# BornToDeath/h264-h265-to-jpeg

Hardware: AMD Instinct MI355X
Metric: 1080p H.265 I-frames/sec → JPEG at 1/2/4/8 MI355X; achieved HBM GB/s vs peak (higher is better)
Workload: dtype u8

## Files before the change

### h264-h265-to-jpeg_amd/csrc/host/bitstream.cpp

```cpp
#include "bitstream.h"

namespace h2j {

void split_annexb(const uint8_t* d, size_t n, std::vector<Nal>& out) {
    out.clear();
    size_t i = 0;
    long start = -1;
    while (i + 2 < n) {
        if (d[i + 2] > 1) {
            i += 3;
            continue;
        }
        if (d[i] == 0 && d[i + 1] == 0 && d[i + 2] == 1) {
            if (start >= 0) {
                size_t e = i;
                while (e > static_cast<size_t>(start) && d[e - 1] == 0) e--;
                out.push_back(Nal{d + start, e - start});
            }
            i += 3;
            start = static_cast<long>(i);
            continue;
        }
        i++;
    }
    if (start >= 0 && static_cast<size_t>(start) < n) {
        size_t e = n;
        while (e > static_cast<size_t>(start) && d[e - 1] == 0) e--;
        out.push_back(Nal{d + start, e - start});
    }
}

size_t unescape_rbsp(const uint8_t* src, size_t n, uint8_t* dst) {
    size_t o = 0;
    int zeros = 0;
    for (size_t i = 0; i < n; i++) {
        uint8_t b = src[i];
        if (zeros >= 2 && b == 3) {
            zeros = 0;
            continue;
        }
        dst[o++] = b;
        zeros = (b == 0) ? zeros + 1 : 0;
    }
    return o;
}

bool BitReader::more_rbsp_data() const {
    long last = static_cast<long>(n_) - 1;
    while (last >= 0 && p_[last] == 0) last--;
    if (last < 0) return false;
    int tz = 0;
    while (!((p_[last] >> tz) & 1)) tz++;
    size_t stop = static_cast<size_t>(last) * 8 + (7 - tz);
    return pos_ < stop;
}

int detect_codec(const uint8_t* d, size_t n) {
    std::vector<Nal> nals;
    split_annexb(d, n < (1u << 16) ? n : (1u << 16), nals);
    int hv = 0, hs = 0, hp = 0, as = 0, ap = 0;
    for (const Nal& nal : nals) {
        if (nal.n < 2) continue;
        uint8_t h0 = nal.p[0], h1 = nal.p[1];
        if (h0 & 0x80) continue;
        int t = (h0 >> 1) & 63, layer = ((h0 & 1) << 5) | (h1 >> 3), tid = h1 & 7;
        if (layer == 0 && tid >= 1) {
            if (t == 32) hv++;
            if (t == 33) hs++;
            if (t == 34) hp++;
        }
        int t4 = h0 & 31;
        if (t4 == 7) as++;
        if (t4 == 8) ap++;
    }
    if (hv && hs && hp) return 265;
    if (as && ap) return 264;
    return 0;
}

int sei_display_orientation(const uint8_t* rbsp, size_t n, bool hevc, int cur) {
    static const uint8_t kCode[2][2][4] = {{{0, 8, 3, 6}, {4, 7, 2, 5}}, {{2, 5, 4, 7}, {3, 6, 0, 8}}};
    (void)hevc;
    size_t pos = 0;
    while (n - pos >= 2) {
        uint32_t type = 0, size = 0;
        while (pos < n && rbsp[pos] == 0xFF && type < (1u << 20)) { type += 255; pos++; }
        if (pos >= n) break;
        type += rbsp[pos++];
        while (pos < n && rbsp[pos] == 0xFF && size < (1u << 20)) { size += 255; pos++; }
        if (pos >= n) {
            if (type == 47) cur = 0;
            break;
        }
        size += rbsp[pos++];
        if (size > n - pos) {
// ... 41 lines not shown
```

### h264-h265-to-jpeg_amd/csrc/host/cabac.h

```cpp
#pragma once
#include <cstdint>

namespace h2j {

#ifdef H2J_CABAC_COUNT
extern thread_local unsigned long long g_bins_ctx, g_bins_byp;
#define H2J_COUNT(v, n) (v += (n))
struct ResidualStats {
    unsigned long long tbs, sb_visited, csbf_bins, sb_coded, sig_bins, sig0_bins, gt1_bins, gt2_bins, last_bins,
        coefs, sb_by_coefs[5] , rem_coefs, rem_sbs, sign_batch_sbs, sign_single_sbs;
    unsigned long long one_coef, one_coef_esc, one_coef_esc_price, one_coef_tskip, one_coef_bypass, one_coef_esc_tskip,
        one_coef_esc_bypass, dc_last_sb, dc_only_tb, sign_pair;
};
extern thread_local ResidualStats g_rstat;
#define H2J_STAT(f, n) (g_rstat.f += (n))
#else
#define H2J_COUNT(v, n) ((void)0)
#define H2J_STAT(f, n) ((void)0)
#endif

#pragma GCC visibility push(hidden)
extern const uint8_t kCabacLps[64][4];
extern const uint8_t kCabacTransLps[64];
extern const uint8_t kCabacRenorm[32];
extern const uint16_t kCabacNextMps[128];
extern const uint16_t kCabacNextLps[128];
extern const uint8_t kCabacLpsByState[128][8];
typedef uint64_t CabacState;
extern const uint64_t kCabacWord[128];

extern const uint64_t kCabacNextMpsW[128];
extern const uint64_t kCabacNextLpsW[128];
#pragma GCC visibility pop


inline uint8_t cabac_init_state(int m, int n, int qp) {
    if (qp < 0) qp = 0;
    if (qp > 51) qp = 51;
    int pre = ((m * qp) >> 4) + n;
    if (pre < 1) pre = 1;
    if (pre > 126) pre = 126;
    int mps = pre <= 63 ? 0 : 1;
    int st = mps ? pre - 64 : 63 - pre;
    return static_cast<uint8_t>((st << 1) | mps);
}
inline CabacState cabac_init_word(int m, int n, int qp) { return kCabacWord[cabac_init_state(m, n, qp)]; }

template <bool kInlineRefill>
class CabacT {
public:
    void init(const uint8_t* p, const uint8_t* end) {
        cur_ = p;
        end_ = end;
        range_ = 510;
        value_ = 0;
        for (int i = 0; i < 4; i++) value_ = (value_ << 8) | (cur_ < end_ ? *cur_++ : 0u);
        bits_ = 32 - 9;
    }
    __attribute__((always_inline)) inline int decision(CabacState& ctx) {
        H2J_COUNT(g_bins_ctx, 1);
        const uint64_t w = ctx;
        const unsigned st = static_cast<unsigned>(w >> 32);
        const uint32_t lps = static_cast<uint32_t>(w >> ((range_ >> 3) & 24)) & 0xffu;
        const uint32_t rmps = range_ - lps;
        const uint64_t scaled = static_cast<uint64_t>(rmps) << bits_;
        const uint32_t msh = (rmps >> 8) ^ 1u;
        uint32_t r = rmps << msh, sh = msh;
        const uint32_t lsh = static_cast<uint32_t>(__builtin_clz(lps)) - 23u;
        const uint32_t lr = lps << lsh;
        uint64_t nx = kCabacNextMpsW[st];
        const uint64_t nl = kCabacNextLpsW[st];
        uint64_t v = value_;
        const uint64_t vl = value_ - scaled;
        uint32_t is_lps = 0;
#if defined(__x86_64__)
        __asm__("cmpq %[sc], %[v]\n\t"
                "cmovaeq %[vl], %[v]\n\t"
                "cmovael %[lr], %[r]\n\t"
                "cmovael %[ls], %[sh]\n\t"
                "cmovaeq %[nl], %[nx]\n\t"
                "setae %b[il]"
                : [v] "+r"(v), [r] "+r"(r), [sh] "+r"(sh), [nx] "+r"(nx), [il] "+q"(is_lps)
                : [sc] "r"(scaled), [vl] "r"(vl), [lr] "r"(lr), [ls] "r"(lsh), [nl] "r"(nl)
                : "cc");
#else
        is_lps = v >= scaled ? 1u : 0u;
        v = is_lps ? vl : v;
        r = is_lps ? lr : r;
        sh = is_lps ? lsh : sh;
        nx = is_lps ? nl : nx;
#endif
        value_ = v;
        range_ = r;
        bits_ -= static_cast<int>(sh);
        ctx = nx;
        if (bits_ < 0) refill();
        return static_cast<int>((st & 1) ^ is_lps);
    }
    __attribute__((always_inline)) int bypass_b() {
        H2J_COUNT(g_bins_byp, 1);
        if (--bits_ < 0) refill();
        const uint64_t scaled = static_cast<uint64_t>(range_) << bits_;
        const bool one = value_ >= scaled;
        value_ -= one ? scaled : 0;
        return one;
    }
    __attribute__((always_inline)) uint32_t bypass_batch_b(int k) {
        H2J_COUNT(g_bins_byp, k);
        if (bits_ < k) refill();
        const int sh = bits_ - k;
        const uint64_t v = value_ >> sh;
        const uint32_t q = static_cast<uint32_t>(v / range_);
        value_ -= (static_cast<uint64_t>(q) * range_) << sh;
        bits_ = sh;
        return q;
    }
    __attribute__((always_inline)) uint32_t bypass_peek_b(int k) {
        if (bits_ < k) refill();
        return static_cast<uint32_t>((value_ >> (bits_ - k)) / range_);
    }
    __attribute__((always_inline)) void bypass_skip_b(int n, uint32_t top) {
        H2J_COUNT(g_bins_byp, n);
        const int sh = bits_ - n;
        value_ -= (static_cast<uint64_t>(top) * range_) << sh;
        bits_ = sh;
    }
    __attribute__((always_inline)) uint32_t bypass_bits_b(int n) {
        if (n <= 2) {
            uint32_t v = 0;
            for (int i = 0; i < n; i++) v = (v << 1) | static_cast<uint32_t>(bypass());
            return v;
        }
        if (n <= 24) return bypass_batch(n);
        const uint32_t hi = bypass_batch(n - 16);
        return (hi << 16) | bypass_batch(16);
    }
    __attribute__((always_inline)) int terminate_b() {
        range_ -= 2;
        const uint64_t scaled = static_cast<uint64_t>(range_) << bits_;
        if (value_ >= scaled) return 1;
        if (range_ < 256) {
            range_ <<= 1;
            if (--bits_ < 0) refill();
        }
        return 0;
    }
    __attribute__((always_inline)) int bypass() { return kInlineRefill ? bypass_b() : bypass_o(); }
    int bypass_o() { return bypass_b(); }
    __attribute__((always_inline)) uint32_t bypass_batch(int k) { return kInlineRefill ? bypass_batch_b(k) : bypass_batch_o(k); }
    uint32_t bypass_batch_o(int k) { return bypass_batch_b(k); }
    __attribute__((always_inline)) uint32_t bypass_peek(int k) { return kInlineRefill ? bypass_peek_b(k) : bypass_peek_o(k); }
    uint32_t bypass_peek_o(int k) { return bypass_peek_b(k); }
    __attribute__((always_inline)) void bypass_skip(int n, uint32_t top) { kInlineRefill ? bypass_skip_b(n, top) : bypass_skip_o(n, top); }
    void bypass_skip_o(int n, uint32_t top) { bypass_skip_b(n, top); }
    __attribute__((always_inline)) uint32_t bypass_bits(int n) { return kInlineRefill ? bypass_bits_b(n) : bypass_bits_o(n); }
    uint32_t bypass_bits_o(int n) { return bypass_bits_b(n); }
    __attribute__((always_inline)) int terminate() { return kInlineRefill ? terminate_b() : terminate_o(); }
    int terminate_o() { return terminate_b(); }
    const uint8_t* aligned_pos() const { return cur_ - (bits_ >> 3); }

private:
    __attribute__((always_inline)) void refill() {
        if (kInlineRefill) refill_word();
        else refill_o();
    }
    void refill_o() {
        uint32_t w;
        if (end_ - cur_ >= 4) {
            w = (static_cast<uint32_t>(cur_[0]) << 24) | (static_cast<uint32_t>(cur_[1]) << 16) |
                (static_cast<uint32_t>(cur_[2]) << 8) | cur_[3];
            cur_ += 4;
        } else {
            w = 0;
            for (int i = 0; i < 4; i++) w = (w << 8) | (cur_ < end_ ? *cur_++ : 0u);
        }
        value_ = (value_ << 32) | w;
        bits_ += 32;
    }
    __attribute__((always_inline)) void refill_word() {
        uint32_t w;
        if (__builtin_expect(end_ - cur_ >= 4, 1)) {
            w = (static_cast<uint32_t>(cur_[0]) << 24) | (static_cast<uint32_t>(cur_[1]) << 16) |
                (static_cast<uint32_t>(cur_[2]) << 8) | cur_[3];
            cur_ += 4;
        } else {
            w = tail_word(cur_, end_);
            cur_ = end_ > cur_ ? end_ : cur_;
        }
        value_ = (value_ << 32) | w;
        bits_ += 32;
    }
    __attribute__((noinline)) static uint32_t tail_word(const uint8_t* cur, const uint8_t* end) {
        uint32_t w = 0;
        for (int i = 0; i < 4; i++) w = (w << 8) | (cur < end ? *cur++ : 0u);
        return w;
    }
    const uint8_t* cur_ = nullptr;
    const uint8_t* end_ = nullptr;
    uint64_t value_ = 0;
    uint32_t range_ = 510;
    int bits_ = 0;
};
typedef CabacT<true> Cabac;
typedef CabacT<false> CabacOutlineRefill;

}
```

### h264-h265-to-jpeg_amd/csrc/host/hevc_parser.cpp

```cpp
#include <algorithm>
#include <array>
#include <atomic>
#include <cstdlib>
#include <cstring>
#include <memory>
#include <thread>
#include <vector>

#include "bitstream.h"
#include "cabac.h"
#include "job.h"

namespace h2j {
namespace {

enum {
    C_SAO_MERGE = 0, C_SAO_TYPE = 1, C_SPLIT_CU = 2, C_TQ_BYPASS = 5, C_PART_MODE = 6,
    C_PREV_INTRA = 7, C_CHROMA_MODE = 8, C_SPLIT_TF = 9, C_CBF_LUMA = 12, C_CBF_CHROMA = 14,
    C_TSKIP = 18, C_LAST_X = 20, C_LAST_Y = 38, C_CSBF = 56, C_SIG = 60, C_GT1 = 104,
    C_GT2 = 128, C_QP_DELTA = 134, C_CQO_FLAG = 136, C_CQO_IDX = 137, NUM_CTX = 138
};

const uint8_t kInitI[NUM_CTX] = {
    153, 200, 139, 141, 157, 154, 184, 184, 63, 153, 138, 138, 111, 141, 94, 138, 182, 154,
// ... 974 lines not shown
}

const uint8_t kSigTs[2][16] = {{C_SIG + 42, C_SIG + 42, C_SIG + 42, C_SIG + 42, C_SIG + 42, C_SIG + 42, C_SIG + 42, C_SIG + 42,
                                C_SIG + 42, C_SIG + 42, C_SIG + 42, C_SIG + 42, C_SIG + 42, C_SIG + 42, C_SIG + 42, C_SIG + 42},
                               {C_SIG + 43, C_SIG + 43, C_SIG + 43, C_SIG + 43, C_SIG + 43, C_SIG + 43, C_SIG + 43, C_SIG + 43,
                                C_SIG + 43, C_SIG + 43, C_SIG + 43, C_SIG + 43, C_SIG + 43, C_SIG + 43, C_SIG + 43, C_SIG + 43}};

__attribute__((always_inline)) inline int read_remaining(Cabac& cc, int rice) {
    constexpr int kPeek = 20;
    const uint32_t q = cc.bypass_peek(kPeek);
    const uint32_t inv = ~q << (32 - kPeek);
    int prefix = inv ? __builtin_clz(inv) : kPeek;
    if (prefix < kPeek) {
        const int slen = prefix < 3 ? rice : prefix - 3 + rice, total = prefix + 1 + slen;
        if (total <= kPeek) {
            const uint32_t top = q >> (kPeek - total);
            cc.bypass_skip(total, top);
            const int suf = static_cast<int>(top & ((1u << slen) - 1u));
            return prefix < 3 ? (prefix << rice) + suf : (((1 << (prefix - 3)) + 2) << rice) + suf;
        }
    }
    prefix = 0;
    while (prefix < 32 && cc.bypass()) prefix++;
    if (prefix < 3) return (prefix << rice) + static_cast<int>(cc.bypass_bits(rice));
    const int pm3 = prefix - 3;
    if (pm3 + rice > 30) return -1;
    return (((1 << pm3) + 2) << rice) + static_cast<int>(cc.bypass_bits(pm3 + rice));
}

__attribute__((noinline)) int HevcParser::remaining_level(int rice) { return read_remaining(cc_, rice); }

template <bool RExt>
void HevcParser::residual(int log2n, int c, int pred_mode, h2j_tu& tu) {
    Cabac cc = cc_;
    CabacState* const ctx = ctx_;
    const int n = 1 << log2n;
    if (p_->transform_skip && !cu_bypass_ && log2n <= (RExt ? p_->log2_max_ts : 2) && cc.decision(ctx[C_TSKIP + (c ? 1 : 0)]))
        tu.flags |= H2J_TU_TSKIP;
    const bool tsb = (tu.flags & H2J_TU_TSKIP) != 0 || cu_bypass_;
    const bool ts_ctx = RExt && s_->ts_context && tsb;
    const bool no_sdh = RExt && s_->implicit_rdpcm && (tu.flags & H2J_TU_TSKIP) && (pred_mode == 10 || pred_mode == 26);
    const bool price = RExt && s_->persistent_rice;
    int* const stat = &stat_[2 * (c == 0 ? 1 : 0) + (tsb ? 1 : 0)];
    int off, shift;
    if (c == 0) {
        off = 3 * (log2n - 2) + ((log2n - 1) >> 2);
        shift = (log2n + 1) >> 2;
    } else {
        off = 15;
        shift = log2n - 2;
    }
    const int maxp = (log2n << 1) - 1;
    H2J_STAT(tbs, 1);
    auto last_prefix = [&](CabacState* lc) __attribute__((always_inline)) {
        int k = 0, pk = 0;
        CabacState pw = lc[0];
        while (k < maxp) {
            const int ci = k >> shift;
            const CabacState lw = lc[ci];
            lc[pk] = pw;
            CabacState w = ci == pk ? pw : lw;
            H2J_STAT(last_bins, 1);
            const int b = cc.decision(w);
            pw = w;
            pk = ci;
            if (!b) break;
            k++;
        }
        lc[pk] = pw;
        return k;
    };
    int lx = last_prefix(ctx + C_LAST_X + off);
    int ly = last_prefix(ctx + C_LAST_Y + off);
    if (lx > 3) {
        int nb = (lx >> 1) - 1;
        lx = (1 << nb) * (2 + (lx & 1)) + static_cast<int>(cc.bypass_bits(nb));
    }
    if (ly > 3) {
        int nb = (ly >> 1) - 1;
        ly = (1 << nb) * (2 + (ly & 1)) + static_cast<int>(cc.bypass_bits(nb));
    }
    int scanIdx = 0;
    if (log2n == 2 || (log2n == 3 && c == 0)) {
        if (pred_mode >= 6 && pred_mode <= 14) scanIdx = 2;
        else if (pred_mode >= 22 && pred_mode <= 30) scanIdx = 1;
    }
    if (scanIdx == 2) std::swap(lx, ly);
    if (lx >= n || ly >= n) { err_ = -20; cc_ = cc; return; }
    const uint8_t(*sc)[64][2] = scanIdx == 0 ? g_scan_diag : (scanIdx == 1 ? g_scan_hor : g_scan_ver);
    const int lsb = log2n - 2;
    const int lastSub = g_scan_inv[scanIdx][lsb][((ly >> 2) << lsb) + (lx >> 2)];
    const int lastPos = g_scan_inv[scanIdx][2][((ly & 3) << 2) + (lx & 3)];
    uint64_t csbm = 0;
    H2J_STAT(dc_only_tb, (lx | ly) == 0);
    int greater1_ctx = 1;
    const bool sdh = p_->sign_hiding != 0;
    uint32_t out[32 * 32];
    int nout = 0;
    const uint16_t* const posTab = g_scan_off[scanIdx][lsb];
    const uint8_t(*const sigtab)[2][16] = g_sigctx[c ? 1 : 0][lsb][scanIdx];
    CabacState* const gt1ctx = ctx + C_GT1 + (c ? 16 : 0);
    for (int i = lastSub; i >= 0; i--) {
        const int xs = sc[lsb][i][0], ys = sc[lsb][i][1];
        H2J_STAT(sb_visited, 1);
        bool infer_dc = false;
        const int sp = ys * 8 + xs;
        const unsigned csr = static_cast<unsigned>(((csbm >> 1) & 0x7f7f7f7f7f7f7f7full) >> sp) & 1u;
        const unsigned csb = static_cast<unsigned>((csbm >> 8) >> sp) & 1u;
        unsigned coded = 1;
        if (i < lastSub && i > 0) {
            H2J_STAT(csbf_bins, 1);
            coded = static_cast<unsigned>(cc.decision(ctx[C_CSBF + (csr | csb) + (c ? 2 : 0)]));
            infer_dc = true;
        }
        csbm |= static_cast<uint64_t>(coded) << sp;
        const int prevCsbf = static_cast<int>(csr | (csb << 1));
        unsigned sigmask = 0;
        int nstart = 15;
        if (i == lastSub) {
            nstart = lastPos - 1;
            sigmask = 1u << lastPos;
            H2J_STAT(dc_last_sb, lastPos == 0);
        }
        if (coded && nstart >= 0) {
            const uint8_t* sig = ts_ctx ? kSigTs[c ? 1 : 0] : sigtab[prevCsbf][(xs | ys) ? 1 : 0];
            unsigned got = 0;
            if (nstart > 0) {
                H2J_STAT(sig_bins, nstart);
                int pidx = sig[nstart];
                CabacState pw = ctx[pidx];
                got = static_cast<unsigned>(cc.decision(pw)) << nstart;
                for (int nn = nstart - 1; nn > 0; nn--) {
                    const int idx = sig[nn];
                    const CabacState lw = ctx[idx];
                    ctx[pidx] = pw;
                    CabacState w = idx == pidx ? pw : lw;
                    got |= static_cast<unsigned>(cc.decision(w)) << nn;
                    pw = w;
                    pidx = idx;
                }
                ctx[pidx] = pw;
            }
            sigmask |= got;
            if (infer_dc && got == 0) {
                sigmask |= 1u;
            } else {
                H2J_STAT(sig0_bins, 1);
                if (cc.decision(ctx[sig[0]])) sigmask |= 1u;
            }
        }
        if (!sigmask) continue;
        H2J_STAT(sb_coded, 1);
        int ctxSet = (i == 0 || c > 0) ? 0 : 2;
        if (greater1_ctx == 0) ctxSet++;
        const int sb_off = ((ys << 2) << log2n) + (xs << 2);
#ifdef H2J_CABAC_COUNT
        {
            const int nc = __builtin_popcount(sigmask);
            H2J_STAT(coefs, nc);
            H2J_STAT(sb_by_coefs[nc == 1 ? 0 : nc == 2 ? 1 : nc == 3 ? 2 : nc < 8 ? 3 : 4], 1);
            H2J_STAT(gt1_bins, nc < 8 ? nc : 8);
        }
#endif
        if ((sigmask & (sigmask - 1)) == 0) {
            H2J_STAT(one_coef, 1);
            H2J_STAT(sign_single_sbs, 1);
            H2J_STAT(one_coef_tskip, (tu.flags & H2J_TU_TSKIP) != 0);
            H2J_STAT(one_coef_bypass, cu_bypass_ != 0);
            const int g1 = cc.decision(gt1ctx[ctxSet * 4 + 1]);
            greater1_ctx = g1 ^ 1;
            int lvl = 1 + g1, g2 = 0;
            if (g1) {
                H2J_STAT(gt2_bins, 1);
                g2 = cc.decision(ctx[C_GT2 + ctxSet + (c ? 4 : 0)]);
                lvl += g2;
            }
            const int neg = cc.bypass();
            if (g2) {
                H2J_STAT(one_coef_esc, 1);
                H2J_STAT(one_coef_esc_price, price);
                H2J_STAT(one_coef_esc_tskip, (tu.flags & H2J_TU_TSKIP) != 0);
                H2J_STAT(one_coef_esc_bypass, cu_bypass_ != 0);
                H2J_STAT(rem_coefs, 1);
                H2J_STAT(rem_sbs, 1);
                cc_ = cc;
                const int rem = remaining_level(price ? *stat / 4 : 0);
                cc = cc_;
                if (rem < 0) { err_ = -21; return; }
                lvl += rem;
                if (price) {
                    const int ri = *stat / 4;
                    if (rem >= (3 << ri)) ++*stat;
                    else if (2 * rem < (1 << ri) && *stat > 0) --*stat;
                }
            }
            int v = neg ? -lvl : lvl;
            if (v > 32767) v = 32767;
            if (v < -32768) v = -32768;
            out[nout++] = (static_cast<uint32_t>(sb_off + posTab[__builtin_ctz(sigmask)]) << 16) | static_cast<uint16_t>(v);
            continue;
        }
        greater1_ctx = 1;
        unsigned g1mask = 0;
        int numG1 = 0, lastG1 = -1;
        unsigned m_uncoded = 0;
        const int lastSig = 31 - __builtin_clz(sigmask), firstSig = __builtin_ctz(sigmask);
        CabacState* const g1c = gt1ctx + ctxSet * 4;
        {
            CabacState w0 = g1c[0], w1 = g1c[1], w2 = g1c[2], w3 = g1c[3];
            unsigned seen = 0, m = sigmask;
            auto bin = [&](CabacState& slot) __attribute__((always_inline)) {
                const int nn = 31 - __builtin_clz(m);
                m &= ~(1u << nn);
                CabacState w = seen ? w0 : slot;
                const unsigned d = static_cast<unsigned>(cc.decision(w));
                if (seen) w0 = w;
                else slot = w;
                seen |= d;
                g1mask |= d << nn;
                numG1++;
            };
            if (m) bin(w1);
            if (m) bin(w2);
            while (m && numG1 < 8) bin(w3);
            g1c[0] = w0;
            g1c[1] = w1;
            g1c[2] = w2;
            g1c[3] = w3;
            m_uncoded = m;
            greater1_ctx = seen ? 0 : 1;
        }
        if (g1mask) lastG1 = 31 - __builtin_clz(g1mask);
        const bool hidden = !cu_bypass_ && !no_sdh && (lastSig - firstSig > 3);
        int g2 = 0;
        if (lastG1 != -1) {
            H2J_STAT(gt2_bins, 1);
            g2 = cc.decision(ctx[C_GT2 + ctxSet + (c ? 4 : 0)]);
        }
        const unsigned signed_mask = (sdh && hidden) ? (sigmask & ~(1u << firstSig)) : sigmask;
        const int ns = __builtin_popcount(signed_mask);
        H2J_STAT(sign_batch_sbs, ns > 1);
        H2J_STAT(sign_single_sbs, ns <= 1);
        H2J_STAT(sign_pair, ns == 2);
        const uint32_t q = ns > 2 ? cc.bypass_batch(ns) : cc.bypass_bits(ns);
        uint32_t qs = ns ? q << (32 - ns) : 0u;
        unsigned esc = g1mask | m_uncoded;
        if (lastG1 >= 0 && !g2) esc &= ~(1u << lastG1);
        H2J_STAT(rem_coefs, __builtin_popcount(esc));
        H2J_STAT(rem_sbs, esc != 0);
        int remv[16] = {};
        int rice = price ? *stat / 4 : 0;
        bool stat_done = false;
        for (unsigned e = esc; e;) {
            const int nn = 31 - __builtin_clz(e);
            e &= ~(1u << nn);
            const int baseL = 1 + ((g1mask >> nn) & 1) + (nn == lastG1 ? g2 : 0);
            const int rem = read_remaining(cc, rice);
            if (rem < 0) { err_ = -21; cc_ = cc; return; }
            remv[nn] = rem;
            if (baseL + rem > 3 * (1 << rice)) rice = price ? rice + 1 : (rice < 4 ? rice + 1 : 4);
            if (price && !stat_done) {
                const int ri = *stat / 4;
                if (rem >= (3 << ri)) ++*stat;
                else if (2 * rem < (1 << ri) && *stat > 0) --*stat;
                stat_done = true;
            }
        }
        const int flip_last = (sdh && hidden) ? 1 : 0;
        int sumAbs = 0;
        for (unsigned mm = sigmask; mm;) {
            const int nn = 31 - __builtin_clz(mm);
            mm &= ~(1u << nn);
            const int lvl = 1 + ((g1mask >> nn) & 1) + (nn == lastG1 ? g2 : 0) + remv[nn];
            sumAbs += lvl;
            const int neg = static_cast<int>(qs >> 31) ^ (mm == 0 ? (flip_last & sumAbs) : 0);
            qs <<= 1;
            int v = neg ? -lvl : lvl;
            if (v > 32767) v = 32767;
            if (v < -32768) v = -32768;
            out[nout++] = (static_cast<uint32_t>(sb_off + posTab[nn]) << 16) | static_cast<uint16_t>(v);
        }
    }
    cc_ = cc;
    const uint32_t base = static_cast<uint32_t>(job_->coefs.size());
    job_->coefs.insert(job_->coefs.end(), out, out + nout);
    tu.coef = base - job_->hdr.coef;
    tu.ncoef = static_cast<uint16_t>(nout);
    tu.flags |= H2J_TU_CBF;
}

void HevcParser::split_ctb_records(size_t first) {
    std::vector<h2j_tu>& v = job_->tus;
    chroma_tmp_.clear();
    size_t w = first;
    for (size_t i = first; i < v.size(); i++) {
        if (v[i].c == 0) v[w++] = v[i];
        else chroma_tmp_.push_back(v[i]);
    }
    std::copy(chroma_tmp_.begin(), chroma_tmp_.end(), v.begin() + static_cast<long>(w));
}

void HevcParser::emit_tu(int x, int y, int log2n, int c, int mode, uint8_t flags, bool cbf, int) {
    job_->tus.emplace_back();
    h2j_tu& tu = job_->tus.back();
    tu.x = static_cast<uint16_t>(x);
    tu.y = static_cast<uint16_t>(y);
    tu.log2n = static_cast<uint8_t>(log2n);
    tu.c = static_cast<uint8_t>(c);
    tu.mode = static_cast<uint8_t>(mode);
    tu.flags = flags;
    tu.qp = 0;
    tu.qpy = 0;
    tu.ncoef = 0;
    tu.coef = 0;
    if (cbf) {
        if (rext_) residual<true>(log2n, c, mode, tu);
        else residual<false>(log2n, c, mode, tu);
    }
}

void HevcParser::transform_unit(int x0, int y0, int xb, int yb, int log2n, int blk, int cbf_l, int cbf_cb,
                                int cbf_cr, int cm, int cux, int cuy, int log2cb) {
    if ((cbf_l || cbf_cb || cbf_cr) && p_->cu_qp_delta && !is_qpd_coded_) {
        int v = 0;
        if (dec(C_QP_DELTA)) {
            v = 1;
            while (v < 5 && dec(C_QP_DELTA + 1)) v++;
            if (v == 5) {
                int k = 0;
                while (k < 32 && cc_.bypass()) k++;
                if (k > 30) { err_ = -22; return; }
                v += ((1 << k) - 1) + static_cast<int>(cc_.bypass_bits(k));
            }
        }
        if (v && cc_.bypass()) v = -v;
        is_qpd_coded_ = true;
        qpd_val_ = v;
        qp_y_ = qp_wrap(qg_pred_ + v + 52 + 2 * qpbd) - qpbd;
        set_qp(cux, cuy, 1 << log2cb, qp_y_);
    }
    if ((cbf_cb || cbf_cr) && cur_->cu_chroma_qp_offset_enabled && !cu_bypass_ && !cqo_coded_) {
        int idx = -1;
        if (dec(C_CQO_FLAG)) {
            idx = 0;
            if (p_->cqo_len_minus1 > 0)
                while (idx < 5 && dec(C_CQO_IDX)) idx++;
        }
        cu_qo_cb_ = idx < 0 ? 0 : p_->cb_qo[idx];
        cu_qo_cr_ = idx < 0 ? 0 : p_->cr_qo[idx];
        cqo_coded_ = true;
    }
    const int lmode = ipm_[(y0 >> 2) * mw + (x0 >> 2)];
    uint8_t fl = edge_flags(x0, y0);
    if (cu_bypass_) fl |= H2J_TU_BYPASS | H2J_TU_NOFILT;
    uint8_t lfl = fl;
    if (log2n == 2) lfl |= H2J_TU_DST;
    emit_tu(x0, y0, log2n, 0, lmode, lfl, cbf_l != 0, lmode);
    if ((job_->tus.back().flags & (H2J_TU_TSKIP | H2J_TU_BYPASS)) != 0) job_->tus.back().flags &= ~H2J_TU_DST;
    if (err_) return;
    uint8_t cfl = cu_bypass_ ? (H2J_TU_BYPASS | H2J_TU_NOFILT) : 0;
    if (log2n > 2) {
        emit_tu(x0 >> 1, y0 >> 1, log2n - 1, 1, cm, cfl, cbf_cb != 0, cm);
        if (err_) return;
        emit_tu(x0 >> 1, y0 >> 1, log2n - 1, 2, cm, cfl, cbf_cr != 0, cm);
    } else if (blk == 3) {
        emit_tu(xb >> 1, yb >> 1, 2, 1, cm, cfl, cbf_cb != 0, cm);
        if (err_) return;
        emit_tu(xb >> 1, yb >> 1, 2, 2, cm, cfl, cbf_cr != 0, cm);
    }
}

void HevcParser::transform_tree(int x0, int y0, int xb, int yb, int log2n, int depth, int blk, int max_depth,
                                int intra_split, int pcb, int pcr, int cm, int cux, int cuy, int log2cb) {
    if (err_) return;
    int split;
    if (log2n <= s_->log2_max_tb && log2n > s_->log2_min_tb && depth < max_depth && !(intra_split && depth == 0))
        split = dec(C_SPLIT_TF + 5 - log2n);
    else
        split = log2n > s_->log2_max_tb || (intra_split && depth == 0);
    int cbf_cb = 0, cbf_cr = 0;
    if (log2n > 2) {
        if (depth == 0 || pcb) cbf_cb = dec(C_CBF_CHROMA + depth);
        if (depth == 0 || pcr) cbf_cr = dec(C_CBF_CHROMA + depth);
    } else {
        cbf_cb = pcb;
        cbf_cr = pcr;
    }
    if (split) {
        if (log2n <= 2) { err_ = -23; return; }
        int h = 1 << (log2n - 1);
        transform_tree(x0, y0, x0, y0, log2n - 1, depth + 1, 0, max_depth, intra_split, cbf_cb, cbf_cr, cm, cux, cuy, log2cb);
        transform_tree(x0 + h, y0, x0, y0, log2n - 1, depth + 1, 1, max_depth, intra_split, cbf_cb, cbf_cr, cm, cux, cuy, log2cb);
        transform_tree(x0, y0 + h, x0, y0, log2n - 1, depth + 1, 2, max_depth, intra_split, cbf_cb, cbf_cr, cm, cux, cuy, log2cb);
        transform_tree(x0 + h, y0 + h, x0, y0, log2n - 1, depth + 1, 3, max_depth, intra_split, cbf_cb, cbf_cr, cm, cux, cuy, log2cb);
    } else {
        int cbf_l = dec(C_CBF_LUMA + (depth == 0 ? 1 : 0));
        transform_unit(x0, y0, xb, yb, log2n, blk, cbf_l, cbf_cb, cbf_cr, cm, cux, cuy, log2cb);
    }
}

void HevcParser::pcm_sample(int x0, int y0, int log2cb) {
    const uint8_t* p = cc_.aligned_pos();
    BitReader b(p, static_cast<size_t>(end_ - p));
    const int n = 1 << log2cb;
    const int bd = s_->bit_depth;
    uint8_t fl = edge_flags(x0, y0) | H2J_TU_PCM | H2J_TU_CBF;
    if (s_->pcm_lf_disabled) fl |= H2J_TU_NOFILT;
    for (int c = 0; c < 3; c++) {
        const int cn = c ? n / 2 : n;
        h2j_tu tu;
        tu.x = static_cast<uint16_t>(c ? x0 / 2 : x0);
        tu.y = static_cast<uint16_t>(c ? y0 / 2 : y0);
        const int sub = cn > 32 ? 32 : cn;
        for (int sy = 0; sy < cn; sy += sub)
            for (int sx = 0; sx < cn; sx += sub) {
                h2j_tu t = tu;
                t.x = static_cast<uint16_t>(tu.x + sx);
                t.y = static_cast<uint16_t>(tu.y + sy);
                t.log2n = static_cast<uint8_t>(sub == 32 ? 5 : (sub == 16 ? 4 : (sub == 8 ? 3 : 2)));
                t.c = static_cast<uint8_t>(c);
                t.mode = 1;
                t.flags = c == 0 ? fl : static_cast<uint8_t>(H2J_TU_PCM | H2J_TU_CBF | (fl & H2J_TU_NOFILT));
                if (c == 0 && (sx || sy)) {
                    t.flags = static_cast<uint8_t>((t.flags & ~(H2J_TU_EDGE_L | H2J_TU_EDGE_T)) |
                                                   (edge_flags(x0 + sx, y0 + sy) & ((sx ? 0 : H2J_TU_EDGE_L) | (sy ? 0 : H2J_TU_EDGE_T))));
                }
                t.qp = 0;
                t.qpy = 0;
                t.coef = static_cast<uint32_t>(job_->coefs.size()) - job_->hdr.coef;
                t.ncoef = static_cast<uint16_t>(sub * sub);
                job_->tus.push_back(t);
                for (int k = 0; k < sub * sub; k++) job_->coefs.push_back(0);
            }
    }
    size_t tu_end = job_->tus.size();
    int recs_y = (n > 32) ? 4 : 1;
    size_t first = tu_end - static_cast<size_t>(recs_y + 2);
    for (int c = 0; c < 3; c++) {
        const int cn = c ? n / 2 : n;
        const int pbd = c ? s_->pcm_bd_c : s_->pcm_bd;
        const int sub = cn > 32 ? 32 : cn;
        for (int y = 0; y < cn; y++)
            for (int x = 0; x < cn; x++) {
                int v = static_cast<int>(b.u(pbd)) << (bd - pbd);
                size_t rec = first + (c == 0 ? static_cast<size_t>((y / sub) * (cn / sub) + x / sub) : static_cast<size_t>(recs_y + c - 1));
                const h2j_tu& t = job_->tus[rec];
                int pos = (y % sub) * sub + (x % sub);
                job_->coefs[job_->hdr.coef + t.coef + pos] = (static_cast<uint32_t>(pos) << 16) | static_cast<uint16_t>(v);
            }
    }
    cc_.init(p + b.byte_pos(), end_);
}

void HevcParser::coding_unit(int x0, int y0, int log2cb) {
    const int n = 1 << log2cb;
    cu_tu_begin_ = static_cast<int>(job_->tus.size());
    cu_bypass_ = 0;
    if (p_->transquant_bypass) cu_bypass_ = dec(C_TQ_BYPASS);
    int part_nxn = 0;
    if (log2cb == s_->log2_min_cb) part_nxn = !dec(C_PART_MODE);
    qp_y_ = qp_wrap(qg_pred_ + qpd_val_ + 52 + 2 * qpbd) - qpbd;
    set_qp(x0, y0, n, qp_y_);
    int pcm = 0;
    if (!part_nxn && s_->pcm && log2cb >= s_->log2_min_pcm && log2cb <= s_->log2_max_pcm) pcm = cc_.terminate();
    if (pcm) {
        set_map(ipm_, x0, y0, n, 1);
        pcm_sample(x0, y0, log2cb);
    } else {
        const int np = part_nxn ? 4 : 1, pb = part_nxn ? n / 2 : n;
        int prev[4], mpm[4] = {0, 0, 0, 0}, rem[4] = {0, 0, 0, 0};
        for (int i = 0; i < np; i++) prev[i] = dec(C_PREV_INTRA);
        for (int i = 0; i < np; i++) {
            if (prev[i]) {
                if (cc_.bypass()) mpm[i] = cc_.bypass() ? 2 : 1;
            } else {
                rem[i] = static_cast<int>(cc_.bypass_bits(5));
            }
        }
        for (int i = 0; i < np; i++) {
            const int xp = x0 + (i & 1) * pb, yp = y0 + (i >> 1) * pb;
            int ca = 1, cb = 1;
            if (same_region(xp, yp, xp - 1, yp)) ca = ipm_[(yp >> 2) * mw + ((xp - 1) >> 2)];
            if (same_region(xp, yp, xp, yp - 1) && ((yp - 1) >> log2ctb) == (yp >> log2ctb))
                cb = ipm_[((yp - 1) >> 2) * mw + (xp >> 2)];
            int cand[3];
            if (ca == cb) {
                if (ca < 2) { cand[0] = 0; cand[1] = 1; cand[2] = 26; }
                else { cand[0] = ca; cand[1] = 2 + ((ca + 29) % 32); cand[2] = 2 + ((ca - 2 + 1) % 32); }
            } else {
                cand[0] = ca;
                cand[1] = cb;
                cand[2] = (ca != 0 && cb != 0) ? 0 : ((ca != 1 && cb != 1) ? 1 : 26);
            }
            int mode;
            if (prev[i]) {
                mode = cand[mpm[i]];
            } else {
                if (cand[0] > cand[1]) std::swap(cand[0], cand[1]);
                if (cand[0] > cand[2]) std::swap(cand[0], cand[2]);
                if (cand[1] > cand[2]) std::swap(cand[1], cand[2]);
                mode = rem[i];
                for (int k = 0; k < 3; k++)
                    if (mode >= cand[k]) mode++;
            }
            set_map(ipm_, xp, yp, pb, static_cast<uint8_t>(mode));
        }
        int icpm = 4;
        if (dec(C_CHROMA_MODE)) icpm = static_cast<int>(cc_.bypass_bits(2));
        const int lm = ipm_[(y0 >> 2) * mw + (x0 >> 2)];
        int cm;
        if (icpm == 4) cm = lm;
        else {
            static const int cmodes[4] = {0, 26, 10, 1};
            cm = cmodes[icpm] == lm ? 34 : cmodes[icpm];
        }
        transform_tree(x0, y0, x0, y0, log2cb, 0, 0, s_->max_th_depth_intra + part_nxn, part_nxn, 0, 0, cm, x0, y0, log2cb);
    }
    const int qpy = qp_y_ + qpbd;
    int qpc[2];
    for (int k = 0; k < 2; k++) {
        int off = k == 0 ? p_->cb_qp_offset + cur_->cb_qp_offset + cu_qo_cb_
                         : p_->cr_qp_offset + cur_->cr_qp_offset + cu_qo_cr_;
        int qpi = qp_y_ + off;
        if (qpi < -qpbd) qpi = -qpbd;
        if (qpi > 57) qpi = 57;
        qpc[k] = chroma_qp_table(qpi) + qpbd;
    }
    for (size_t t = static_cast<size_t>(cu_tu_begin_); t < job_->tus.size(); t++) {
        h2j_tu& tu = job_->tus[t];
        tu.qpy = static_cast<int8_t>(qp_y_);
        tu.qp = static_cast<int8_t>(tu.c == 0 ? qpy : qpc[tu.c - 1]);
    }
    last_cu_qp_ = qp_y_;
}

void HevcParser::coding_quadtree(int x0, int y0, int log2cb, int depth) {
    if (err_) return;
    const int n = 1 << log2cb;
    int split;
    if (x0 + n <= W && y0 + n <= H && log2cb > s_->log2_min_cb) {
        int inc = 0;
        if (same_region(x0, y0, x0 - 1, y0) && ctd_[(y0 >> 2) * mw + ((x0 - 1) >> 2)] > depth) inc++;
        if (same_region(x0, y0, x0, y0 - 1) && ctd_[((y0 - 1) >> 2) * mw + (x0 >> 2)] > depth) inc++;
        split = dec(C_SPLIT_CU + inc);
    } else {
        split = log2cb > s_->log2_min_cb;
    }
    if ((p_->cu_qp_delta && log2cb >= log2ctb - p_->diff_cu_qp_delta_depth) || (!p_->cu_qp_delta && log2cb == log2ctb))
        qg_start(x0, y0);
    if (cur_->cu_chroma_qp_offset_enabled && log2cb >= log2ctb - p_->cqo_depth) cqo_coded_ = false;
    if (split) {
        const int h = n >> 1;
        coding_quadtree(x0, y0, log2cb - 1, depth + 1);
        if (x0 + h < W) coding_quadtree(x0 + h, y0, log2cb - 1, depth + 1);
        if (y0 + h < H) coding_quadtree(x0, y0 + h, log2cb - 1, depth + 1);
        if (x0 + h < W && y0 + h < H) coding_quadtree(x0 + h, y0 + h, log2cb - 1, depth + 1);
    } else {
        set_map(ctd_, x0, y0, n, static_cast<uint8_t>(depth));
        coding_unit(x0, y0, log2cb);
    }
}

void HevcParser::ctb_start_contexts(int rs, int ts, bool first) {
    const int rx = rs % ctbW;
    const int x0 = rx << log2ctb, y0 = (rs / ctbW) << log2ctb;
    const bool tile_start = ts == 0 || tile_id_[ts] != tile_id_[ts - 1];
    bool row_start = false;
    if (p_->wpp)
        for (size_t i = 0; i + 1 < col_bd_.size(); i++)
            if (rx == col_bd_[i]) row_start = true;
    if (!(first || tile_start || row_start)) return;
    if (tile_start) {
        init_contexts(cur_->slice_qp);
    } else if (row_start) {
        const int xr = x0 + ctbs, yr = y0 - ctbs;
        if (xr < W && yr >= 0 && same_region(x0, y0, xr, yr)) {
            std::memcpy(ctx_, ctx_wpp_, sizeof(ctx_));
            std::memcpy(stat_, stat_wpp_, sizeof(stat_));
        } else {
            init_contexts(cur_->slice_qp);
        }
    } else if (cur_->dependent && have_ds_) {
        std::memcpy(ctx_, ctx_ds_, sizeof(ctx_));
        std::memcpy(stat_, stat_ds_, sizeof(stat_));
    } else {
        init_contexts(cur_->slice_qp);
    }
    if (tile_start || row_start) {
        first_qg_ = true;
        last_cu_qp_ = cur_->slice_qp;
    }
}

int HevcParser::decode_slice_data(int shi, const uint8_t* p, const uint8_t* end) {
    const SliceHdr& sh = sh_[shi];
    cur_ = &sh;
    cur_idx_ = shi;
    end_ = end;
    cc_.init(p, end);
    int rs = sh.address, ts = rs2ts_[rs];
    if (!sh.dependent) {
        first_qg_ = true;
        last_cu_qp_ = sh.slice_qp;
        cu_qo_cb_ = cu_qo_cr_ = 0;
// ... 371 lines not shown
```

Before: 2175.

## Speed up host bitstream scanning and CABAC residual decode, add branch-site profiling

Start-code splitting and emulation-prevention removal now use memchr and memcpy instead of byte-by-byte loops. The CABAC reader gains a branchless 32-bit top-up that is called once per sub-block. Uncoded sub-blocks now skip their body early, and the coefficient output loop is unrolled by four with a padded output buffer. Branch-site profiling counters are added, but they compile to plain conditions unless the counting build flag is set. The top-up logic and the unrolled output that relies on the padding are correctness-sensitive, and host-side parsing may not be the throughput bottleneck.

```diff
diff --git a/h264-h265-to-jpeg_amd/csrc/host/bitstream.cpp b/h264-h265-to-jpeg_amd/csrc/host/bitstream.cpp
--- a/h264-h265-to-jpeg_amd/csrc/host/bitstream.cpp
+++ b/h264-h265-to-jpeg_amd/csrc/host/bitstream.cpp
@@ -1,46 +1,50 @@
 #include "bitstream.h"
+
+#include <cstring>
 
 namespace h2j {
 
 void split_annexb(const uint8_t* d, size_t n, std::vector<Nal>& out) {
     out.clear();
+    long start = -1;
+    auto close = [&](size_t e) {
+        while (e > static_cast<size_t>(start) && d[e - 1] == 0) e--;
+        out.push_back(Nal{d + start, e - static_cast<size_t>(start)});
+    };
     size_t i = 0;
-    long start = -1;
     while (i + 2 < n) {
-        if (d[i + 2] > 1) {
-            i += 3;
-            continue;
+        const uint8_t* one = static_cast<const uint8_t*>(std::memchr(d + i + 2, 1, n - (i + 2)));
+        if (!one) break;
+        const size_t j = static_cast<size_t>(one - d);
+        if (d[j - 1] == 0 && d[j - 2] == 0) {
+            if (start >= 0) close(j - 2);
+            i = j + 1;
+            start = static_cast<long>(i);
+        } else {
+            i = j - 1;
         }
-        if (d[i] == 0 && d[i + 1] == 0 && d[i + 2] == 1) {
-            if (start >= 0) {
-                size_t e = i;
-                while (e > static_cast<size_t>(start) && d[e - 1] == 0) e--;
-                out.push_back(Nal{d + start, e - start});
-            }
-            i += 3;
-            start = static_cast<long>(i);
-            continue;
-        }
-        i++;
     }
-    if (start >= 0 && static_cast<size_t>(start) < n) {
-        size_t e = n;
-        while (e > static_cast<size_t>(start) && d[e - 1] == 0) e--;
-        out.push_back(Nal{d + start, e - start});
-    }
+    if (start >= 0 && static_cast<size_t>(start) < n) close(n);
 }
 
 size_t unescape_rbsp(const uint8_t* src, size_t n, uint8_t* dst) {
-    size_t o = 0;
-    int zeros = 0;
-    for (size_t i = 0; i < n; i++) {
-        uint8_t b = src[i];
-        if (zeros >= 2 && b == 3) {
-            zeros = 0;
-            continue;
+    size_t o = 0, seg = 0, from = 2;
+    while (from < n) {
+        const uint8_t* three = static_cast<const uint8_t*>(std::memchr(src + from, 3, n - from));
+        if (!three) break;
+        const size_t j = static_cast<size_t>(three - src);
+        if (src[j - 1] == 0 && src[j - 2] == 0) {
+            std::memcpy(dst + o, src + seg, j - seg);
+            o += j - seg;
+            seg = j + 1;
+            from = seg + 2;
+        } else {
+            from = j + 1;
         }
-        dst[o++] = b;
-        zeros = (b == 0) ? zeros + 1 : 0;
+    }
+    if (seg < n) {
+        std::memcpy(dst + o, src + seg, n - seg);
+        o += n - seg;
     }
     return o;
 }
diff --git a/h264-h265-to-jpeg_amd/csrc/host/cabac.h b/h264-h265-to-jpeg_amd/csrc/host/cabac.h
--- a/h264-h265-to-jpeg_amd/csrc/host/cabac.h
+++ b/h264-h265-to-jpeg_amd/csrc/host/cabac.h
@@ -14,9 +14,51 @@
 };
 extern thread_local ResidualStats g_rstat;
 #define H2J_STAT(f, n) (g_rstat.f += (n))
+#define H2J_BRANCH_SITES(X)                                                                               \
+    X(last_x_max) X(last_x_bin) X(last_y_max) X(last_y_bin) X(last_x_suffix) X(last_y_suffix)             \
+    X(sub_block_loop) X(csbf_coded_range) X(sub_block_uncoded) X(is_last_sub_block) X(sig_scan)           \
+    X(sig_scan_bins) X(sig_loop) X(infer_dc) X(sub_block_empty) X(one_coef_split) X(one_coef_g1)          \
+    X(one_coef_g2) X(g1_second_bin) X(g1_loop) X(g1_any) X(signs_gt2) X(escape_loop) X(output_loop)       \
+    X(decision_refill) X(bypass_refill) X(tt_split_coded) X(tt_split) X(tt_chroma_cbf_read)               \
+    X(tt_cbf_cb_coded) X(tt_cbf_cr_coded) X(tu_qp_delta) X(tu_chroma_blocks) X(tu_chroma_4x4) X(tb_cbf)   \
+    X(cu_part_coded) X(cu_prev_intra) X(cu_mpm_idx0) X(cu_mpm_idx1) X(cu_cand_equal) X(cu_cand_lt2)       \
+    X(cu_cand_sort) X(cu_rem_ge_cand) X(cu_chroma_mode) X(cu_qp_patch_loop) X(cq_split_coded)             \
+    X(cq_split)
+enum BranchSite {
+#define H2J_X(n) BS_##n,
+    H2J_BRANCH_SITES(H2J_X)
+#undef H2J_X
+    BS_COUNT
+};
+struct BranchSiteStat {
+    unsigned long long exec, taken, miss;
+    unsigned state;
+};
+extern thread_local BranchSiteStat g_bsite[BS_COUNT];
+inline bool branch_site(BranchSite s, bool taken) {
+    BranchSiteStat& b = g_bsite[s];
+    const unsigned st = b.state ^ 1u;
+    b.exec++;
+    b.taken += taken;
+    b.miss += (st >= 2) != taken;
+    b.state = (taken ? (st < 3 ? st + 1 : 3u) : (st > 0 ? st - 1 : 0u)) ^ 1u;
+    return taken;
+}
+#ifdef H2J_NO_BRANCH_SITES
+#define H2J_BR(site, cond) (cond)
+#else
+#define H2J_BR(site, cond) (::h2j::branch_site(::h2j::BS_##site, (cond)))
+#endif
 #else
 #define H2J_COUNT(v, n) ((void)0)
 #define H2J_STAT(f, n) ((void)0)
+#define H2J_BR(site, cond) (cond)
+#endif
+
+#if defined(__clang__)
+#define H2J_UNPREDICTABLE(c) __builtin_unpredictable(c)
+#else
+#define H2J_UNPREDICTABLE(c) (c)
 #endif
 
 #pragma GCC visibility push(hidden)
@@ -94,12 +136,12 @@
         range_ = r;
         bits_ -= static_cast<int>(sh);
         ctx = nx;
-        if (bits_ < 0) refill();
+        if (H2J_BR(decision_refill, bits_ < 0)) refill();
         return static_cast<int>((st & 1) ^ is_lps);
     }
     __attribute__((always_inline)) int bypass_b() {
         H2J_COUNT(g_bins_byp, 1);
-        if (--bits_ < 0) refill();
+        if (H2J_BR(bypass_refill, --bits_ < 0)) refill();
         const uint64_t scaled = static_cast<uint64_t>(range_) << bits_;
         const bool one = value_ >= scaled;
         value_ -= one ? scaled : 0;
@@ -157,6 +199,18 @@
     uint32_t bypass_bits_o(int n) { return bypass_bits_b(n); }
     __attribute__((always_inline)) int terminate() { return kInlineRefill ? terminate_b() : terminate_o(); }
     int terminate_o() { return terminate_b(); }
+    __attribute__((always_inline)) void top_up() {
+        if (__builtin_expect(end_ - cur_ < 4, 0)) return;
+        static_assert(__BYTE_ORDER__ == __ORDER_LITTLE_ENDIAN__, "the word load below swaps a little-endian word");
+        uint32_t w;
+        __builtin_memcpy(&w, cur_, 4);
+        w = __builtin_bswap32(w);
+        const bool need = bits_ < 24;
+        const uint64_t nv = (value_ << 32) | w;
+        value_ = H2J_UNPREDICTABLE(need) ? nv : value_;
+        bits_ += H2J_UNPREDICTABLE(need) ? 32 : 0;
+        cur_ += H2J_UNPREDICTABLE(need) ? 4 : 0;
+    }
     const uint8_t* aligned_pos() const { return cur_ - (bits_ >> 3); }
 
 private:
diff --git a/h264-h265-to-jpeg_amd/csrc/host/hevc_parser.cpp b/h264-h265-to-jpeg_amd/csrc/host/hevc_parser.cpp
--- a/h264-h265-to-jpeg_amd/csrc/host/hevc_parser.cpp
+++ b/h264-h265-to-jpeg_amd/csrc/host/hevc_parser.cpp
@@ -1050,10 +1050,11 @@
     }
     const int maxp = (log2n << 1) - 1;
     H2J_STAT(tbs, 1);
-    auto last_prefix = [&](CabacState* lc) __attribute__((always_inline)) {
+    auto last_prefix = [&](CabacState* lc, bool is_y) __attribute__((always_inline)) {
+        (void)is_y;
         int k = 0, pk = 0;
         CabacState pw = lc[0];
-        while (k < maxp) {
+        while (is_y ? H2J_BR(last_y_max, k < maxp) : H2J_BR(last_x_max, k < maxp)) {
             const int ci = k >> shift;
             const CabacState lw = lc[ci];
             lc[pk] = pw;
@@ -1062,19 +1063,19 @@
             const int b = cc.decision(w);
             pw = w;
             pk = ci;
-            if (!b) break;
+            if (is_y ? H2J_BR(last_y_bin, !b) : H2J_BR(last_x_bin, !b)) break;
             k++;
         }
         lc[pk] = pw;
         return k;
     };
-    int lx = last_prefix(ctx + C_LAST_X + off);
-    int ly = last_prefix(ctx + C_LAST_Y + off);
-    if (lx > 3) {
+    int lx = last_prefix(ctx + C_LAST_X + off, false);
+    int ly = last_prefix(ctx + C_LAST_Y + off, true);
+    if (H2J_BR(last_x_suffix, lx > 3)) {
         int nb = (lx >> 1) - 1;
         lx = (1 << nb) * (2 + (lx & 1)) + static_cast<int>(cc.bypass_bits(nb));
     }
-    if (ly > 3) {
+    if (H2J_BR(last_y_suffix, ly > 3)) {
         int nb = (ly >> 1) - 1;
         ly = (1 << nb) * (2 + (ly & 1)) + static_cast<int>(cc.bypass_bits(nb));
     }
@@ -1093,42 +1094,44 @@
     H2J_STAT(dc_only_tb, (lx | ly) == 0);
     int greater1_ctx = 1;
     const bool sdh = p_->sign_hiding != 0;
-    uint32_t out[32 * 32];
+    uint32_t out[32 * 32 + 4];
     int nout = 0;
     const uint16_t* const posTab = g_scan_off[scanIdx][lsb];
     const uint8_t(*const sigtab)[2][16] = g_sigctx[c ? 1 : 0][lsb][scanIdx];
     CabacState* const gt1ctx = ctx + C_GT1 + (c ? 16 : 0);
-    for (int i = lastSub; i >= 0; i--) {
+    for (int i = lastSub; H2J_BR(sub_block_loop, i >= 0); i--) {
         const int xs = sc[lsb][i][0], ys = sc[lsb][i][1];
+        cc.top_up();
         H2J_STAT(sb_visited, 1);
         bool infer_dc = false;
         const int sp = ys * 8 + xs;
         const unsigned csr = static_cast<unsigned>(((csbm >> 1) & 0x7f7f7f7f7f7f7f7full) >> sp) & 1u;
         const unsigned csb = static_cast<unsigned>((csbm >> 8) >> sp) & 1u;
         unsigned coded = 1;
-        if (i < lastSub && i > 0) {
+        if (H2J_BR(csbf_coded_range, i < lastSub && i > 0)) {
             H2J_STAT(csbf_bins, 1);
             coded = static_cast<unsigned>(cc.decision(ctx[C_CSBF + (csr | csb) + (c ? 2 : 0)]));
             infer_dc = true;
         }
         csbm |= static_cast<uint64_t>(coded) << sp;
+        if (H2J_BR(sub_block_uncoded, !coded)) continue;
         const int prevCsbf = static_cast<int>(csr | (csb << 1));
         unsigned sigmask = 0;
         int nstart = 15;
-        if (i == lastSub) {
+        if (H2J_BR(is_last_sub_block, i == lastSub)) {
             nstart = lastPos - 1;
             sigmask = 1u << lastPos;
             H2J_STAT(dc_last_sb, lastPos == 0);
         }
-        if (coded && nstart >= 0) {
+        if (H2J_BR(sig_scan, nstart >= 0)) {
             const uint8_t* sig = ts_ctx ? kSigTs[c ? 1 : 0] : sigtab[prevCsbf][(xs | ys) ? 1 : 0];
             unsigned got = 0;
-            if (nstart > 0) {
+            if (H2J_BR(sig_scan_bins, nstart > 0)) {
                 H2J_STAT(sig_bins, nstart);
                 int pidx = sig[nstart];
                 CabacState pw = ctx[pidx];
                 got = static_cast<unsigned>(cc.decision(pw)) << nstart;
-                for (int nn = nstart - 1; nn > 0; nn--) {
+                for (int nn = nstart - 1; H2J_BR(sig_loop, nn > 0); nn--) {
                     const int idx = sig[nn];
                     const CabacState lw = ctx[idx];
                     ctx[pidx] = pw;
@@ -1140,14 +1143,14 @@
                 ctx[pidx] = pw;
             }
             sigmask |= got;
-            if (infer_dc && got == 0) {
+            if (H2J_BR(infer_dc, infer_dc && got == 0)) {
                 sigmask |= 1u;
             } else {
                 H2J_STAT(sig0_bins, 1);
                 if (cc.decision(ctx[sig[0]])) sigmask |= 1u;
             }
         }
-        if (!sigmask) continue;
+        if (H2J_BR(sub_block_empty, !sigmask)) continue;
         H2J_STAT(sb_coded, 1);
         int ctxSet = (i == 0 || c > 0) ? 0 : 2;
         if (greater1_ctx == 0) ctxSet++;
@@ -1160,7 +1163,7 @@
             H2J_STAT(gt1_bins, nc < 8 ? nc : 8);
         }
 #endif
-        if ((sigmask & (sigmask - 1)) == 0) {
+        if (H2J_BR(one_coef_split, (sigmask & (sigmask - 1)) == 0)) {
             H2J_STAT(one_coef, 1);
             H2J_STAT(sign_single_sbs, 1);
             H2J_STAT(one_coef_tskip, (tu.flags & H2J_TU_TSKIP) != 0);
@@ -1168,13 +1171,13 @@
             const int g1 = cc.decision(gt1ctx[ctxSet * 4 + 1]);
             greater1_ctx = g1 ^ 1;
             int lvl = 1 + g1, g2 = 0;
-            if (g1) {
+            if (H2J_BR(one_coef_g1, g1 != 0)) {
                 H2J_STAT(gt2_bins, 1);
                 g2 = cc.decision(ctx[C_GT2 + ctxSet + (c ? 4 : 0)]);
                 lvl += g2;
             }
             const int neg = cc.bypass();
-            if (g2) {
+            if (H2J_BR(one_coef_g2, g2 != 0)) {
                 H2J_STAT(one_coef_esc, 1);
                 H2J_STAT(one_coef_esc_price, price);
                 H2J_STAT(one_coef_esc_tskip, (tu.flags & H2J_TU_TSKIP) != 0);
@@ -1219,8 +1222,8 @@
                 numG1++;
             };
             if (m) bin(w1);
-            if (m) bin(w2);
-            while (m && numG1 < 8) bin(w3);
+            if (H2J_BR(g1_second_bin, m != 0)) bin(w2);
+            while (H2J_BR(g1_loop, m && numG1 < 8)) bin(w3);
             g1c[0] = w0;
             g1c[1] = w1;
             g1c[2] = w2;
@@ -1231,7 +1234,7 @@
         if (g1mask) lastG1 = 31 - __builtin_clz(g1mask);
         const bool hidden = !cu_bypass_ && !no_sdh && (lastSig - firstSig > 3);
         int g2 = 0;
-        if (lastG1 != -1) {
+        if (H2J_BR(g1_any, lastG1 != -1)) {
             H2J_STAT(gt2_bins, 1);
             g2 = cc.decision(ctx[C_GT2 + ctxSet + (c ? 4 : 0)]);
         }
@@ -1240,7 +1243,7 @@
         H2J_STAT(sign_batch_sbs, ns > 1);
         H2J_STAT(sign_single_sbs, ns <= 1);
         H2J_STAT(sign_pair, ns == 2);
-        const uint32_t q = ns > 2 ? cc.bypass_batch(ns) : cc.bypass_bits(ns);
+        const uint32_t q = H2J_BR(signs_gt2, ns > 2) ? cc.bypass_batch(ns) : cc.bypass_bits(ns);
         uint32_t qs = ns ? q << (32 - ns) : 0u;
         unsigned esc = g1mask | m_uncoded;
         if (lastG1 >= 0 && !g2) esc &= ~(1u << lastG1);
@@ -1249,7 +1252,7 @@
         int remv[16] = {};
         int rice = price ? *stat / 4 : 0;
         bool stat_done = false;
-        for (unsigned e = esc; e;) {
+        for (unsigned e = esc; H2J_BR(escape_loop, e != 0);) {
             const int nn = 31 - __builtin_clz(e);
             e &= ~(1u << nn);
             const int baseL = 1 + ((g1mask >> nn) & 1) + (nn == lastG1 ? g2 : 0);
@@ -1266,8 +1269,10 @@
         }
         const int flip_last = (sdh && hidden) ? 1 : 0;
         int sumAbs = 0;
-        for (unsigned mm = sigmask; mm;) {
-            const int nn = 31 - __builtin_clz(mm);
+        unsigned mm = sigmask;
+        uint32_t* o = out + nout;
+        auto entry = [&]() __attribute__((always_inline)) {
+            const int nn = 31 - __builtin_clz(mm | 1u);
             mm &= ~(1u << nn);
             const int lvl = 1 + ((g1mask >> nn) & 1) + (nn == lastG1 ? g2 : 0) + remv[nn];
             sumAbs += lvl;
@@ -1276,8 +1281,15 @@
             int v = neg ? -lvl : lvl;
             if (v > 32767) v = 32767;
             if (v < -32768) v = -32768;
-            out[nout++] = (static_cast<uint32_t>(sb_off + posTab[nn]) << 16) | static_cast<uint16_t>(v);
-        }
+            *o++ = (static_cast<uint32_t>(sb_off + posTab[nn]) << 16) | static_cast<uint16_t>(v);
+        };
+        do {
+            entry();
+            entry();
+            entry();
+            entry();
+        } while (H2J_BR(output_loop, mm != 0));
+        nout += __builtin_popcount(sigmask);
     }
     cc_ = cc;
     const uint32_t base = static_cast<uint32_t>(job_->coefs.size());
@@ -1311,7 +1323,7 @@
     tu.qpy = 0;
     tu.ncoef = 0;
     tu.coef = 0;
-    if (cbf) {
+    if (H2J_BR(tb_cbf, cbf)) {
         if (rext_) residual<true>(log2n, c, mode, tu);
         else residual<false>(log2n, c, mode, tu);
     }
@@ -1319,7 +1331,7 @@
 
 void HevcParser::transform_unit(int x0, int y0, int xb, int yb, int log2n, int blk, int cbf_l, int cbf_cb,
                                 int cbf_cr, int cm, int cux, int cuy, int log2cb) {
-    if ((cbf_l || cbf_cb || cbf_cr) && p_->cu_qp_delta && !is_qpd_coded_) {
+    if (H2J_BR(tu_qp_delta, (cbf_l || cbf_cb || cbf_cr) && p_->cu_qp_delta && !is_qpd_coded_)) {
         int v = 0;
         if (dec(C_QP_DELTA)) {
             v = 1;
@@ -1357,11 +1369,11 @@
     if ((job_->tus.back().flags & (H2J_TU_TSKIP | H2J_TU_BYPASS)) != 0) job_->tus.back().flags &= ~H2J_TU_DST;
     if (err_) return;
     uint8_t cfl = cu_bypass_ ? (H2J_TU_BYPASS | H2J_TU_NOFILT) : 0;
-    if (log2n > 2) {
+    if (H2J_BR(tu_chroma_blocks, log2n > 2)) {
         emit_tu(x0 >> 1, y0 >> 1, log2n - 1, 1, cm, cfl, cbf_cb != 0, cm);
         if (err_) return;
         emit_tu(x0 >> 1, y0 >> 1, log2n - 1, 2, cm, cfl, cbf_cr != 0, cm);
-    } else if (blk == 3) {
+    } else if (H2J_BR(tu_chroma_4x4, blk == 3)) {
         emit_tu(xb >> 1, yb >> 1, 2, 1, cm, cfl, cbf_cb != 0, cm);
         if (err_) return;
         emit_tu(xb >> 1, yb >> 1, 2, 2, cm, cfl, cbf_cr != 0, cm);
@@ -1372,19 +1384,19 @@
                                 int intra_split, int pcb, int pcr, int cm, int cux, int cuy, int log2cb) {
     if (err_) return;
     int split;
-    if (log2n <= s_->log2_max_tb && log2n > s_->log2_min_tb && depth < max_depth && !(intra_split && depth == 0))
+    if (H2J_BR(tt_split_coded, log2n <= s_->log2_max_tb && log2n > s_->log2_min_tb && depth < max_depth && !(intra_split && depth == 0)))
         split = dec(C_SPLIT_TF + 5 - log2n);
     else
         split = log2n > s_->log2_max_tb || (intra_split && depth == 0);
     int cbf_cb = 0, cbf_cr = 0;
-    if (log2n > 2) {
-        if (depth == 0 || pcb) cbf_cb = dec(C_CBF_CHROMA + depth);
-        if (depth == 0 || pcr) cbf_cr = dec(C_CBF_CHROMA + depth);
+    if (H2J_BR(tt_chroma_cbf_read, log2n > 2)) {
+        if (H2J_BR(tt_cbf_cb_coded, depth == 0 || pcb)) cbf_cb = dec(C_CBF_CHROMA + depth);
+        if (H2J_BR(tt_cbf_cr_coded, depth == 0 || pcr)) cbf_cr = dec(C_CBF_CHROMA + depth);
     } else {
         cbf_cb = pcb;
         cbf_cr = pcr;
     }
-    if (split) {
+    if (H2J_BR(tt_split, split != 0)) {
         if (log2n <= 2) { err_ = -23; return; }
         int h = 1 << (log2n - 1);
         transform_tree(x0, y0, x0, y0, log2n - 1, depth + 1, 0, max_depth, intra_split, cbf_cb, cbf_cr, cm, cux, cuy, log2cb);
@@ -1456,7 +1468,7 @@
     cu_bypass_ = 0;
     if (p_->transquant_bypass) cu_bypass_ = dec(C_TQ_BYPASS);
     int part_nxn = 0;
-    if (log2cb == s_->log2_min_cb) part_nxn = !dec(C_PART_MODE);
+    if (H2J_BR(cu_part_coded, log2cb == s_->log2_min_cb)) part_nxn = !dec(C_PART_MODE);
     qp_y_ = qp_wrap(qg_pred_ + qpd_val_ + 52 + 2 * qpbd) - qpbd;
     set_qp(x0, y0, n, qp_y_);
     int pcm = 0;
@@ -1469,8 +1481,8 @@
         int prev[4], mpm[4] = {0, 0, 0, 0}, rem[4] = {0, 0, 0, 0};
         for (int i = 0; i < np; i++) prev[i] = dec(C_PREV_INTRA);
         for (int i = 0; i < np; i++) {
-            if (prev[i]) {
-                if (cc_.bypass()) mpm[i] = cc_.bypass() ? 2 : 1;
+            if (H2J_BR(cu_prev_intra, prev[i] != 0)) {
+                if (H2J_BR(cu_mpm_idx0, cc_.bypass() != 0)) mpm[i] = H2J_BR(cu_mpm_idx1, cc_.bypass() != 0) ? 2 : 1;
             } else {
                 rem[i] = static_cast<int>(cc_.bypass_bits(5));
             }
@@ -1482,8 +1494,8 @@
             if (same_region(xp, yp, xp, yp - 1) && ((yp - 1) >> log2ctb) == (yp >> log2ctb))
                 cb = ipm_[((yp - 1) >> 2) * mw + (xp >> 2)];
             int cand[3];
-            if (ca == cb) {
-                if (ca < 2) { cand[0] = 0; cand[1] = 1; cand[2] = 26; }
+            if (H2J_BR(cu_cand_equal, ca == cb)) {
+                if (H2J_BR(cu_cand_lt2, ca < 2)) { cand[0] = 0; cand[1] = 1; cand[2] = 26; }
                 else { cand[0] = ca; cand[1] = 2 + ((ca + 29) % 32); cand[2] = 2 + ((ca - 2 + 1) % 32); }
             } else {
                 cand[0] = ca;
@@ -1494,17 +1506,17 @@
             if (prev[i]) {
                 mode = cand[mpm[i]];
             } else {
-                if (cand[0] > cand[1]) std::swap(cand[0], cand[1]);
-                if (cand[0] > cand[2]) std::swap(cand[0], cand[2]);
-                if (cand[1] > cand[2]) std::swap(cand[1], cand[2]);
+                if (H2J_BR(cu_cand_sort, cand[0] > cand[1])) std::swap(cand[0], cand[1]);
+                if (H2J_BR(cu_cand_sort, cand[0] > cand[2])) std::swap(cand[0], cand[2]);
+                if (H2J_BR(cu_cand_sort, cand[1] > cand[2])) std::swap(cand[1], cand[2]);
                 mode = rem[i];
                 for (int k = 0; k < 3; k++)
-                    if (mode >= cand[k]) mode++;
+                    if (H2J_BR(cu_rem_ge_cand, mode >= cand[k])) mode++;
             }
             set_map(ipm_, xp, yp, pb, static_cast<uint8_t>(mode));
         }
         int icpm = 4;
-        if (dec(C_CHROMA_MODE)) icpm = static_cast<int>(cc_.bypass_bits(2));
+        if (H2J_BR(cu_chroma_mode, dec(C_CHROMA_MODE) != 0)) icpm = static_cast<int>(cc_.bypass_bits(2));
         const int lm = ipm_[(y0 >> 2) * mw + (x0 >> 2)];
         int cm;
         if (icpm == 4) cm = lm;
@@ -1524,7 +1536,7 @@
         if (qpi > 57) qpi = 57;
         qpc[k] = chroma_qp_table(qpi) + qpbd;
     }
-    for (size_t t = static_cast<size_t>(cu_tu_begin_); t < job_->tus.size(); t++) {
+    for (size_t t = static_cast<size_t>(cu_tu_begin_); H2J_BR(cu_qp_patch_loop, t < job_->tus.size()); t++) {
         h2j_tu& tu = job_->tus[t];
         tu.qpy = static_cast<int8_t>(qp_y_);
         tu.qp = static_cast<int8_t>(tu.c == 0 ? qpy : qpc[tu.c - 1]);
@@ -1536,7 +1548,7 @@
     if (err_) return;
     const int n = 1 << log2cb;
     int split;
-    if (x0 + n <= W && y0 + n <= H && log2cb > s_->log2_min_cb) {
+    if (H2J_BR(cq_split_coded, x0 + n <= W && y0 + n <= H && log2cb > s_->log2_min_cb)) {
         int inc = 0;
         if (same_region(x0, y0, x0 - 1, y0) && ctd_[(y0 >> 2) * mw + ((x0 - 1) >> 2)] > depth) inc++;
         if (same_region(x0, y0, x0, y0 - 1) && ctd_[((y0 - 1) >> 2) * mw + (x0 >> 2)] > depth) inc++;
@@ -1547,7 +1559,7 @@
     if ((p_->cu_qp_delta && log2cb >= log2ctb - p_->diff_cu_qp_delta_depth) || (!p_->cu_qp_delta && log2cb == log2ctb))
         qg_start(x0, y0);
     if (cur_->cu_chroma_qp_offset_enabled && log2cb >= log2ctb - p_->cqo_depth) cqo_coded_ = false;
-    if (split) {
+    if (H2J_BR(cq_split, split != 0)) {
         const int h = n >> 1;
         coding_quadtree(x0, y0, log2cb - 1, depth + 1);
         if (x0 + h < W) coding_quadtree(x0 + h, y0, log2cb - 1, depth + 1);
```

New measurement: 2236, median of 6. 2.8% higher.
